# Bismarrck/tensoralloy

Measured on AMD Instinct MI355X. Metric: atom-steps/sec (energy+forces), 4000-atom Ni rcut=6.5 A, higher is better.
Workload: dtype f64

## Files before the change

### tensoralloy_amd/csrc/ta_api.hip

```cpp
#include <hip/hip_runtime.h>

#include <algorithm>
#include <chrono>
#include <climits>
#include <cmath>
#include <cstdio>
#include <cstdlib>
#include <cstring>
#include <stdexcept>
#include <string>
#include <vector>

#include "ta_device.h"
#include "ta_internal.h"
#include "ta_md.h"

namespace ta {
size_t mlp_scratch_doubles(const MlpDev &mlp);
void launch_mlp_impl(const MlpDev &mlp, int activation, int ndim, const int32_t *atoms, int n_atoms,
                     const DeviceBatch &b, double *scratch, hipStream_t s);
size_t mlp_all_scratch_doubles(const MlpDev *mlps_host, int nel, const int32_t *elem_start);
size_t td_scratch_doubles(const MlpDev *nets, int nel, int K, const int32_t *elem_start);
void launch_td_all(const MlpDev *nets_dev, const MlpDev *nets_host, int nel, int K, int act_h, int act,
                   int sommerfeld, int ndim, const DeviceBatch &b, const double *T, double *u_atom,
// ... 172 lines not shown
    if (n <= cap) return;
    if (ptr) HIP_CHECK(hipHostFree(ptr));
    ptr = nullptr;
    cap = 0;
    size_t want = n + n / 8 + 256;
    HIP_CHECK(hipHostMalloc((void **)&ptr, want, hipHostMallocDefault));
    cap = want;
  }
  void release() {
    if (ptr) (void)hipHostFree(ptr);
    ptr = nullptr;
    cap = 0;
  }
};

struct ChunkPlan {
  ta::AngChunk ch;
  int nb, ng, nz;
};

}

struct ta_context {
  int device = 0;
  hipStream_t stream = nullptr;
  hipStream_t own_stream = nullptr;
  int kind = 0;
  int n_elements = 0;
  int activation = 0;
  double rmax = 0.0;
  ta::SFParams sf;
  std::vector<ChunkPlan> chunks;
  std::vector<ChunkPlan> chunks_v2;
  bool use_v2 = false;
  ta::MlpDev *mlp_dev = nullptr;
  ta::MlpDev mlp[ta::kMaxElements];
  bool td = false, td_sommerfeld = false;
  int td_act = 0, td_K = 0;
  ta::MlpDev td_nets[3 * ta::kMaxElements];
  ta::MlpDev *td_dev = nullptr;
  std::vector<void *> model_allocs;
  ta::EamModel *eam = nullptr;
  ta::GrapModel *grap = nullptr;

  ta::HostPairs hp;
  ta::DeviceBatch db;
  bool have_batch = false;
  uint32_t last_want = 0;

  PinnedBuf stage_in, stage_out;
  DevBuf<char> inbuf;
  DevBuf<double> results;
  size_t o_blk = 0;
  DevBuf<double> rec, part4, G, dEdG, g, wat, bpart, fown, benergy, mlp_scratch;
  DevBuf<double> td_T, td_u, td_s;
  DevBuf<unsigned long long> masks;
  DevBuf<uint32_t> job_word;
  DevBuf<int32_t> job_count;
  DevBuf<uint32_t> job_word_own;
  DevBuf<int32_t> job_count_own;
  bool triangles = true;
  bool tri_cells_ok = false;
  int last_bwd_variant = 0;
  DevBuf<int32_t> pair_start, seg_start, pair_i, pair_j, pair_shift, pair_rev;
  ta::NlGrid *d_grids = nullptr;
  DevBuf<int32_t> nl_wrap, nl_binid, nl_bin_count, nl_bin_start, nl_bin_cursor, nl_bin_atoms, nl_counts;
  DevBuf<unsigned long long> nl_stats, nl_zero;
  unsigned long long *nl_stats_ptr = nullptr;
  bool nl_sorted = false;
  bool nl_rev_done = false;
  bool nl_zero_clean = false;
  int64_t nl_zero_atoms = -1;
  int nl_zero_bins = -1;
  DevBuf<double> hvp_buf;
#ifdef TA_PHASE_STAMPS
  DevBuf<unsigned long long> stamp_buf;
#endif
  DevBuf<ta::NlRec> nl_recs;
  bool pairs_on_device = false;
  bool descriptors_valid = false;
  DevBuf<double> train_scratch, train_partial, train_grad, train_coeff;
  DevBuf<double> jvp_J, tan_dD, tan_dG, tan_dir;
  DevBuf<double> filt_scratch;
  bool jvp_valid = false;

  double skin = 0.0;
  double r_list = 0.0;
  std::vector<int32_t> keep_species;
  std::vector<int32_t> keep_natoms, keep_pbc;
  std::vector<double> ref_pos, ref_cells;
  size_t o_pos = 0, o_cells = 0, o_species = 0;
  DevBuf<int32_t> ex_pair_i, ex_pair_j, ex_pair_shift, ex_pair_rev, ex_pair_start, ex_pair_stop, ex_seg_start, ex_counts,
      ex_map, ex_blk, ex_slot_q;
  bool filtered = false;
  bool upload_pending = false;
  bool mirror_next = false;
  uint32_t mirror_want = 0;
  int64_t n_list_builds = 0, n_list_reuses = 0;

  bool md_valid = false;
  DevBuf<double> md_mass, md_vel, md_ref, md_epot, md_ke;
  DevBuf<int32_t> md_blk_start;
  DevBuf<unsigned> md_status;
  PinnedBuf md_status_host;
  std::vector<int32_t> md_blk_start_host;
  int md_chunk = 0, md_n_blk = 0;
  int64_t md_ref_builds = -1;
// ... 456 lines not shown
  using namespace ta;
  if (h->nl_sorted) {
    nl_reverse_sorted(h->hp.n_pairs, h->n_elements, h->db.species, h->seg_start.ptr, h->pair_i.ptr,
                      h->pair_j.ptr, h->pair_shift.ptr, h->pair_rev.ptr, h->nl_stats_ptr, h->stream);
  } else {
    NlWork w = nl_work(h);
    nl_fill((int)h->hp.n_atoms, h->hp.n_pairs, h->n_elements, h->r_list, h->db.pos, h->db.species,
            h->db.frame_of_atom, h->d_grids, w, h->pair_i.ptr, h->pair_j.ptr, h->pair_shift.ptr,
            h->pair_rev.ptr, h->stream);
  }
  HIP_CHECK(hipGetLastError());
}

#ifdef TA_PHASE_STAMPS
static void dump_stamps(ta_context *h) {
  const char *path = std::getenv("TA_PHASE_STAMPS_OUT");
  if (!path || !h->db.stamps || h->db.n_blk <= 0) return;
  const size_t n = (size_t)2 * h->db.n_blk * 8;
  std::vector<unsigned long long> v(n);
  (void)hipStreamSynchronize(h->stream);
  (void)hipMemcpy(v.data(), h->db.stamps, n * sizeof(unsigned long long), hipMemcpyDeviceToHost);
  FILE *fp = std::fopen(path, "w");
  if (!fp) return;
  for (int k = 0; k < 2; ++k)
    for (int b = 0; b < h->db.n_blk; ++b) {
      std::fprintf(fp, "%d %d", k, b);
      for (int q = 0; q < 8; ++q) std::fprintf(fp, " %llu", v[((size_t)k * h->db.n_blk + b) * 8 + q]);
      std::fprintf(fp, "\n");
    }
  std::fclose(fp);
}
#endif

void launch_head(ta_context *h, const ta::DeviceBatch &db, hipStream_t s) {
  if (h->td)
    ta::launch_td_all(h->td_dev, h->td_nets, h->n_elements, h->td_K, h->td_act, h->activation,
                      h->td_sommerfeld ? 1 : 0, h->sf.ndim, db, h->td_T.ptr, h->td_u.ptr, h->td_s.ptr,
                      h->mlp_scratch.ptr, s);
  else
    ta::launch_mlp_all(h->mlp_dev, h->mlp, h->n_elements, h->activation, h->sf.ndim, db, h->mlp_scratch.ptr, s);
}

void compute_impl(ta_context *h, uint32_t want, bool timed, double *slot_ms) {
  using namespace ta;
#ifdef TA_PHASE_STAMPS
  if (h->db.n_blk > 0) {
    h->stamp_buf.ensure((size_t)2 * h->db.n_blk * 8 + 8);
    h->db.stamps = h->stamp_buf.ptr;
    (void)hipMemsetAsync(h->db.stamps, 0, (size_t)2 * h->db.n_blk * 8 * sizeof(unsigned long long), h->stream);
  }
#endif
  h->db.rec4 = nullptr;
  h->db.own_sums = 0;
  const DeviceBatch &db = h->db;
  hipStream_t s = h->stream;
  const bool need_forces = (want & (TA_WANT_FORCES | TA_WANT_VIRIAL)) != 0;
  auto begin = [&](int slot) {
    if (timed) HIP_CHECK(hipEventRecord(h->ev[2 * slot], s));
  };
  auto end = [&](int slot) {
    if (timed) HIP_CHECK(hipEventRecord(h->ev[2 * slot + 1], s));
  };
  bool used[TA_N_KERNEL_SLOTS] = {false};

  const bool has_mlp = h->kind == TA_MODEL_SF_MLP || h->kind == TA_MODEL_GRAP_MLP;
  if ((want & TA_WANT_REUSE_DESCRIPTORS) && has_mlp && h->descriptors_valid && !need_forces) {
    begin(TA_K_MLP);
    launch_head(h, db, s);
    end(TA_K_MLP);
    used[TA_K_MLP] = true;
  } else if (h->kind == TA_MODEL_SF_MLP) {
    static const bool full_records = getenv("TA_FULL_RECORDS") != nullptr;
    h->db.rec4 = (h->sf.angular && h->use_v2 && !full_records) ? h->db.rec : nullptr;
    if (!h->use_v2) {
      begin(TA_K_PAIR_GEOMETRY);
      launch_pair_geometry(h->sf, db, s);
      end(TA_K_PAIR_GEOMETRY);
      used[TA_K_PAIR_GEOMETRY] = true;
    }
    h->sf.ang_scale = h->use_v2 ? 1.0 : 0.5;
    const bool tri = h->use_v2 && h->triangles && h->tri_cells_ok && h->n_elements == 1 && need_forces;
    h->db.job_word_own = (tri && h->db.job_count) ? h->job_word_own.ptr : nullptr;
    h->db.job_count_own = (tri && h->db.job_count) ? h->job_count_own.ptr : nullptr;
    h->last_bwd_variant = 0;
    const bool reduce_in_forward = h->sf.angular && h->use_v2;
    if (h->sf.angular) {
      begin(TA_K_G4_FORWARD);
      if (h->use_v2) {
        bool geometry = true;
        size_t left = h->chunks_v2.size();
        for (const ChunkPlan &cp : h->chunks_v2) {
          --left;
          launch_g4_forward_v2(h->sf, cp.ch, cp.ng, cp.nz, geometry, left == 0, db, s);
          geometry = false;
        }
      } else
        for (const ChunkPlan &cp : h->chunks) launch_g4_forward(h->sf, cp.ch, cp.nb, cp.ng, cp.nz, db, s);
      end(TA_K_G4_FORWARD);
      used[TA_K_G4_FORWARD] = true;
    }
    if (!reduce_in_forward) {
      begin(TA_K_DESCRIPTOR_REDUCE);
      launch_descriptor_reduce(h->sf, db, s);
      end(TA_K_DESCRIPTOR_REDUCE);
      used[TA_K_DESCRIPTOR_REDUCE] = true;
    }
    begin(TA_K_MLP);
    launch_head(h, db, s);
    end(TA_K_MLP);
    used[TA_K_MLP] = true;
    if (need_forces) {
      begin(TA_K_BACKWARD);
      if (h->sf.angular) {
        bool first = true;
        if (h->use_v2)
          for (const ChunkPlan &cp : h->chunks_v2) {
            h->last_bwd_variant |= launch_backward_v2(h->sf, cp.ch, cp.ng, cp.nz, first, tri, db, s);
            first = false;
          }
        else
          for (const ChunkPlan &cp : h->chunks) {
            launch_backward(h->sf, cp.ch, cp.nb, cp.ng, cp.nz, first, false, db, s);
            first = false;
          }
      } else {
        AngChunk dummy;
        std::memset(&dummy, 0, sizeof(dummy));
        launch_backward(h->sf, dummy, 1, 1, 1, true, true, db, s);
      }
      end(TA_K_BACKWARD);
      used[TA_K_BACKWARD] = true;
      begin(TA_K_FORCE_GATHER);
      launch_force_gather(h->sf, db, s);
      end(TA_K_FORCE_GATHER);
      used[TA_K_FORCE_GATHER] = true;
    }
  } else if (h->kind == TA_MODEL_GRAP_MLP) {
    const bool net_exact = ta::grap_uses_filter_net(h->grap) && !ta::grap_filter_table_knots(h->grap);
    h->db.rec4 = (!net_exact && !getenv("TA_FULL_RECORDS")) ? h->db.rec : nullptr;
    begin(TA_K_GRAP);
    launch_grap_forward(h->grap, db, h->sf.eps, s);
    end(TA_K_GRAP);
    used[TA_K_GRAP] = true;
    begin(TA_K_MLP);
    launch_head(h, db, s);
    end(TA_K_MLP);
    used[TA_K_MLP] = true;
    if (need_forces) {
      begin(TA_K_BACKWARD);
      h->db.own_sums = getenv("TA_NO_OWN_SUMS") ? 0 : 1;
      launch_grap_backward(h->grap, db, s);
      end(TA_K_BACKWARD);
      used[TA_K_BACKWARD] = true;
      begin(TA_K_FORCE_GATHER);
      launch_force_gather(h->sf, db, s);
      end(TA_K_FORCE_GATHER);
      used[TA_K_FORCE_GATHER] = true;
    }
  } else {
    h->db.rec4 = getenv("TA_FULL_RECORDS") ? nullptr : h->db.rec;
    begin(TA_K_EAM);
    eam_compute(h->eam, db, want, s, nullptr);
    end(TA_K_EAM);
    used[TA_K_EAM] = true;
  }
  begin(TA_K_FRAME_REDUCE);
  {
    double *mirror = nullptr;
    int64_t n_tail = 0;
    h->mirror_want = 0;
    if (h->mirror_next && !timed) {
      const size_t N = (size_t)db.n_atoms, F = (size_t)db.n_frames;
      h->stage_out.ensure((10 * F + 4 * N + 2) * sizeof(double));
      mirror = reinterpret_cast<double *>(h->stage_out.ptr);
      n_tail = (int64_t)(need_forces ? 4 * N : N);
      h->mirror_want = want | TA_WANT_ENERGY | TA_WANT_ATOMIC;
    }
    launch_frame_reduce(db, need_forces, mirror, n_tail, s);
  }
  end(TA_K_FRAME_REDUCE);
  used[TA_K_FRAME_REDUCE] = true;
  HIP_CHECK(hipGetLastError());
  h->last_want = want;
  h->descriptors_valid = true;

  if (timed) {
    HIP_CHECK(hipStreamSynchronize(s));
    for (int k = 0; k < TA_N_KERNEL_SLOTS; ++k) {
      if (!used[k]) continue;
      float ms = 0.f;
      HIP_CHECK(hipEventElapsedTime(&ms, h->ev[2 * k], h->ev[2 * k + 1]));
      slot_ms[k] += ms;
    }
  }
}

template <typename F>
int guarded(ta_context *h, F &&fn) {
  try {
    if (h) HIP_CHECK(hipSetDevice(h->device));
    fn();
    return TA_OK;
  } catch (const HipError &e) {
    return fail(h, TA_ERR_HIP, e.what());
  } catch (const std::domain_error &e) {
    return fail(h, TA_ERR_UNSUPPORTED, e.what());
  } catch (const std::invalid_argument &e) {
    return fail(h, TA_ERR_INVALID, e.what());
  } catch (const std::bad_alloc &) {
    return fail(h, TA_ERR_NOMEM, "host allocation failed");
  } catch (const std::exception &e) {
    return fail(h, TA_ERR_INVALID, e.what());
  }
}

}

extern "C" {

int ta_abi_version(void) { return TA_ABI_VERSION; }
int ta_model_desc_size(void) { return (int)sizeof(ta_model_desc); }

int ta_device_count(void) {
  int n = 0;
  if (hipGetDeviceCount(&n) != hipSuccess) return 0;
  return n;
}

const char *ta_last_error(ta_handle h) { return h ? h->err.c_str() : g_create_error.c_str(); }

int ta_create(const ta_model_desc *model, int device, ta_handle *out) {
  if (!model || !out) return fail(nullptr, TA_ERR_INVALID, "null argument");
  *out = nullptr;
  int ndev = 0;
// ... 12 lines not shown
    if (std::strncmp(prop.gcnArchName, "gfx950", 6) != 0)
      throw HipError(std::string("device is ") + prop.gcnArchName +
                     ", this library is built for gfx950 only");
    HIP_CHECK(hipStreamCreateWithFlags(&h->own_stream, hipStreamNonBlocking));
    h->stream = h->own_stream;
    for (auto &e : h->ev) HIP_CHECK(hipEventCreate(&e));
    if (model->kind == TA_MODEL_SF_MLP) {
      build_sf_model(h, model);
    } else if (model->kind == TA_MODEL_GRAP_MLP) {
      if (model->cutoff_function != TA_CUTOFF_COSINE && model->cutoff_function != TA_CUTOFF_POLYNOMIAL)
        throw std::invalid_argument("unknown cutoff function");
      std::string err;
      h->grap = ta::grap_create(model, err);
      if (!h->grap) throw std::invalid_argument(err);
      h->rmax = model->rcut;
      std::memset(&h->sf, 0, sizeof(h->sf));
      h->sf.n_elements = model->n_elements;
      h->sf.eps = model->eps > 0.0 ? model->eps : 1e-14;
      h->sf.ndim = ta::grap_ndim(h->grap);
      build_mlp(h, model, h->sf.ndim);
    } else if (model->kind == TA_MODEL_EAM_ALLOY || model->kind == TA_MODEL_EAM_ADP || model->kind == TA_MODEL_EAM_FS) {
      std::string err;
      h->eam = ta::eam_create(model, err);
      if (!h->eam) throw std::invalid_argument(err);
      h->rmax = model->rcut;
      std::memset(&h->sf, 0, sizeof(h->sf));
      h->sf.n_elements = model->n_elements;
      h->sf.eps = model->eps > 0.0 ? model->eps : 1e-14;
    } else {
      throw std::invalid_argument("unknown model kind");
    }
  });
  if (rc != TA_OK) {
    g_create_error = h->err;
    ta_destroy(h);
    return rc;
  }
  *out = h;
  return TA_OK;
}

int ta_destroy(ta_handle h) {
  if (!h) return TA_OK;
  (void)hipSetDevice(h->device);
#ifdef TA_PHASE_STAMPS
  dump_stamps(h);
#endif
  if (h->stream) (void)hipStreamSynchronize(h->stream);
  for (void *p : h->model_allocs) (void)hipFree(p);
  if (h->eam) ta::eam_destroy(h->eam);
  if (h->grap) ta::grap_destroy(h->grap);
  h->stage_in.release(); h->stage_out.release(); h->inbuf.release(); h->results.release();
  h->rec.release(); h->part4.release(); h->G.release();
  h->dEdG.release(); h->g.release(); h->wat.release(); h->bpart.release(); h->fown.release();
  h->benergy.release(); h->mlp_scratch.release();
  h->train_scratch.release(); h->train_partial.release(); h->train_grad.release(); h->train_coeff.release();
  h->jvp_J.release(); h->tan_dD.release(); h->tan_dG.release(); h->tan_dir.release();
  h->pair_start.release(); h->seg_start.release(); h->pair_i.release(); h->pair_j.release();
  h->pair_shift.release(); h->pair_rev.release();
  for (auto *b : {&h->ex_pair_i, &h->ex_pair_j, &h->ex_pair_shift, &h->ex_pair_rev, &h->ex_pair_start, &h->ex_pair_stop,
                  &h->ex_seg_start, &h->ex_counts, &h->ex_map, &h->ex_blk, &h->ex_slot_q})
    b->release();
  h->masks.release(); h->job_word.release(); h->job_count.release();
  h->job_word_own.release(); h->job_count_own.release();
  for (auto *b : {&h->nl_wrap, &h->nl_binid, &h->nl_bin_count, &h->nl_bin_start, &h->nl_bin_cursor,
                  &h->nl_bin_atoms, &h->nl_counts})
    b->release();
  h->nl_stats.release();
  h->nl_zero.release();
  h->hvp_buf.release();
  h->filt_scratch.release();
  h->nl_recs.release();
  for (auto *b : {&h->md_mass, &h->md_vel, &h->md_ref, &h->md_epot, &h->md_ke, &h->md_noise}) b->release();
  h->md_blk_start.release();
  h->md_status.release();
  h->md_status_host.release();
  for (auto &e : h->ev)
    if (e) (void)hipEventDestroy(e);
  if (h->own_stream) (void)hipStreamDestroy(h->own_stream);
  delete h;
  return TA_OK;
}

}

namespace {
void ensure_job_lists(ta_context *h, size_t n_blk) {
  static const bool off = std::getenv("TA_NO_JOBS") != nullptr;
  if (off || !h->use_v2 || n_blk == 0) {
    h->db.job_count = nullptr;
    return;
  }
  const int stride = ta::v2_job_stride(h->db.cap);
  h->job_word.ensure(n_blk * (size_t)stride + 8);
  h->job_count.ensure(n_blk + 8);
  if (h->n_elements == 1) {
    h->job_word_own.ensure(n_blk * (size_t)stride + 8);
    h->job_count_own.ensure(n_blk + 8);
  }
  h->db.job_word = h->job_word.ptr;
  h->db.job_count = h->job_count.ptr;
  h->db.job_stride = stride;
}

bool filter_applies(const ta_context *h) {
  if (!(h->skin > 0.0) || h->hp.n_atoms == 0 || std::getenv("TA_NO_LIST_FILTER")) return false;
  if (h->kind == TA_MODEL_SF_MLP) return h->use_v2;
  if (h->kind == TA_MODEL_EAM_ALLOY || h->kind == TA_MODEL_EAM_FS) return ta::eam_is_plain(h->eam);
  return false;
}

void apply_filter(ta_context *h) {
  using namespace ta;
  const size_t N = (size_t)h->hp.n_atoms, P = (size_t)h->hp.n_pairs;
  const int nel = h->n_elements;
  h->ex_pair_i.ensure(P + 1);
  h->ex_pair_j.ensure(P + 1);
  h->ex_pair_shift.ensure(3 * P + 3);
  h->ex_pair_rev.ensure(P + 1);
  h->ex_pair_start.ensure(N + 1);
  h->ex_pair_stop.ensure(N + 1);
  h->ex_seg_start.ensure(N * (nel + 1) + 1);
  h->ex_map.ensure(P + 1);
  const int n_run_slots = nl_filter_blocks((int)N);
  h->ex_blk.ensure((size_t)n_run_slots + 4);
  const bool blocks = h->kind == TA_MODEL_SF_MLP;
  const bool indirect = blocks && !std::getenv("TA_FILTER_REV_KERNEL");
  if (indirect) h->ex_slot_q.ensure(P + 1);
  nl_filter((int)N, (int64_t)P, nel, h->rmax, h->db.pos, h->db.cells, h->db.frame_of_atom,
            h->pair_start.ptr, h->seg_start.ptr, h->pair_j.ptr, h->pair_shift.ptr, h->pair_rev.ptr, h->ex_map.ptr,
            h->ex_seg_start.ptr, h->ex_pair_start.ptr, h->ex_pair_stop.ptr, h->ex_pair_i.ptr, h->ex_pair_j.ptr,
            h->ex_pair_shift.ptr, h->ex_pair_rev.ptr, indirect ? h->ex_slot_q.ptr : nullptr, h->db.cap,
            blocks ? h->ex_blk.ptr : nullptr, h->stream);
  h->db.slot_q = indirect ? h->ex_slot_q.ptr : nullptr;
  h->db.rev_super = indirect ? h->pair_rev.ptr : nullptr;
  h->db.rev_map = indirect ? h->ex_map.ptr : nullptr;
  HIP_CHECK(hipGetLastError());
  h->db.pair_start = h->ex_pair_start.ptr;
  h->db.pair_stop = h->ex_pair_stop.ptr;
  h->db.seg_start = h->ex_seg_start.ptr;
// ... 1779 lines not shown
```

### tensoralloy_amd/csrc/ta_device.h

```cpp
#pragma once
#include <hip/hip_runtime.h>

#include <cstdint>

#include "tensoralloy_amd.h"

namespace ta {

constexpr int kMaxRadial = 64;
constexpr int kMaxElements = 8;
constexpr int kMaxBetaSlots = 3;
constexpr int kRecDoubles = 8;
constexpr int kMaxLayers = 8;
constexpr int kCapMin = 192;
constexpr int kCapMax = 1024;
constexpr int kMaxCentersPerBlock = 16;
constexpr int kMaxHd = 24;

struct SFParams {
  double rcut, acut;
  double inv_rc2, inv_ac2;
  double two_inv_ac2;
  double eps;
  double ang_scale;
// ... 15 lines not shown
  int hslot[2];
  double gamma[2];
  double zeta[2];
  double kz[2];
  int zeta_int[2];
  int chan[8];
  int safe_pow;
  int n_hd;
  double hd[kMaxHd];
};

struct DeviceBatch {
  int64_t n_atoms = 0, n_pairs = 0;
  int n_frames = 0, nnl_max = 0;
  double *pos = nullptr;
  double *cells = nullptr;
  int32_t *species = nullptr;
  int32_t *frame_of_atom = nullptr;
  int32_t *atom_start = nullptr;
  int32_t *pair_start = nullptr;
  int32_t *pair_stop = nullptr;
  int32_t *seg_start = nullptr;
  int32_t *pair_i = nullptr, *pair_j = nullptr, *pair_shift = nullptr, *pair_rev = nullptr;
  const int32_t *slot_q = nullptr, *rev_super = nullptr, *rev_map = nullptr;
  int32_t *blk_center = nullptr;
  int n_blk = 0;
  int blk_groups = 0;
  const int32_t *n_blk_dev = nullptr;
  int cap = kCapMin;
  int32_t *elem_atoms = nullptr;
  int32_t elem_start[kMaxElements + 1] = {0};

  double *rec = nullptr;
  double *rec4 = nullptr;
  double *part4 = nullptr;
  unsigned long long *masks = nullptr;
  uint32_t *job_word = nullptr;
  int32_t *job_count = nullptr;
  int job_stride = 0;
  uint32_t *job_word_own = nullptr;
  int32_t *job_count_own = nullptr;
  double *G = nullptr;
  double *dEdG = nullptr;
  double *eatom = nullptr;
  double *g = nullptr;
  double *forces = nullptr;
  double *wat = nullptr;
  double *fown = nullptr;
  int own_sums = 0;
#ifdef TA_PHASE_STAMPS
  unsigned long long *stamps = nullptr;
#endif
  double *bpart = nullptr;
  double *energy = nullptr;
  double *virial = nullptr;
  double *batch_energy = nullptr;
};

__host__ __device__ inline int triangle_owner_rank(uint32_t index_sum) {
#ifdef __HIP_DEVICE_COMPILE__
  const uint32_t h = __umul24(index_sum, 0x9E3779u);
#else
  const uint32_t h = index_sum * 0x9E3779u;
#endif
  return (int)(((h & 0xFFFFFFu) * 3u) >> 24);
}
__host__ __device__ inline bool owns_triangle(int32_t i, int32_t j, int32_t k) {
  return triangle_owner_rank((uint32_t)i + (uint32_t)j + (uint32_t)k) == (j < i ? 1 : 0) + (k < i ? 1 : 0);
}

#ifdef __HIPCC__
__device__ __forceinline__ int pair_stop_of(const DeviceBatch &b, int64_t i) {
  return b.pair_stop ? b.pair_stop[i] : b.pair_start[i + 1];
}
#endif

#ifdef __HIPCC__
__device__ __forceinline__ int pair_rev_of(const DeviceBatch &b, int q) {
  return b.slot_q ? b.rev_map[b.rev_super[b.slot_q[q]]] : b.pair_rev[q];
}
__device__ __forceinline__ const double2 *pair_geom(const DeviceBatch &b, size_t q) {
  return reinterpret_cast<const double2 *>(b.rec4 ? b.rec4 + 4 * q : b.rec + kRecDoubles * q);
}
#endif

struct MlpLayerDev {
  int k, n;
  int kp, np;
  double *w;
  double *wt;
  double *b;
  int act;
  int res;
};
struct MlpDev {
  int n_layers = 0;
  MlpLayerDev layer[kMaxLayers];
  double *xlo = nullptr, *xhi = nullptr;
  int max_np = 0, max_kp = 0;
};

void launch_pair_geometry(const SFParams &sf, const DeviceBatch &b, hipStream_t s);
void launch_g4_forward(const SFParams &sf, const AngChunk &ch, int nb, int ng, int nz,
                       const DeviceBatch &b, hipStream_t s);
void launch_descriptor_reduce(const SFParams &sf, const DeviceBatch &b, hipStream_t s);
void launch_mlp(const SFParams &sf, const MlpDev &mlp, int activation, int element,
                const DeviceBatch &b, hipStream_t s);
void launch_backward(const SFParams &sf, const AngChunk &ch, int nb, int ng, int nz,
                     bool first, bool radial_only, const DeviceBatch &b, hipStream_t s);
void launch_force_gather(const SFParams &sf, const DeviceBatch &b, hipStream_t s);
void launch_frame_reduce(const DeviceBatch &b, bool want_virial, double *mirror, int64_t n_tail, hipStream_t s);

size_t g4_lds_bytes(int nnl_max);

size_t v2_lds_bytes(bool backward, int cap, int n_local = 0, int nspec = 0, bool triangles = false);
int v2_job_stride(int cap);
void launch_g4_forward_v2(const SFParams &sf, const AngChunk &ch, int ng, int nz, bool geometry,
                          bool reduce, const DeviceBatch &b, hipStream_t s);
int launch_backward_v2(const SFParams &sf, const AngChunk &ch, int ng, int nz, bool first, bool triangles,
                       const DeviceBatch &b, hipStream_t s);

struct NlGrid {
  double h[9];
  double hinv[9];
  double lo[3];
  double inv_w[3];
  int32_t nb[3];
  int32_t pbc[3];
  int32_t bin_offset;
  int32_t pad_;
  int32_t m[3];
  int32_t ortho;
  double bw[3];
};
struct NlRec {
  double x, y, z;
  int32_t wx, wy, wz;
  int32_t j;
  int32_t sp;
  int32_t pad_;
};
struct NlWork {
  int32_t *wrap;
  int32_t *binid;
  int32_t *bin_count;
  int32_t *bin_start;
  int32_t *bin_cursor;
  int32_t *bin_atoms;
  NlRec *recs;
  int32_t *counts;
  int32_t *seg_start;
  unsigned long long *stats;
};
bool nl_make_grid(const ta_frame &fr, double rmax, int bin_offset, NlGrid &g);
int nl_bins(const NlGrid &g);
void nl_count(int n_atoms, int n_bins, int nel, double rmax, const double *pos, const int32_t *species,
              const int32_t *frame_of_atom, const NlGrid *grids, NlWork &w, int32_t *pair_start,
              hipStream_t s);
size_t nl_build_zero_words(int n_atoms, int n_bins);
void nl_build(int n_atoms, int n_bins, int nel, double rmax, const double *pos, const int32_t *species,
              const int32_t *frame_of_atom, const NlGrid *grids, NlWork &w, unsigned long long *zero,
              bool zero_is_clean, long long capacity, int32_t *pair_start, int32_t *host_pair_start,
              int32_t *pair_i, int32_t *pair_j, int32_t *pair_shift, int32_t *pair_rev, long long rev_cover,
              hipStream_t s);
void nl_reverse_sorted(int64_t n_pairs, int nel, const int32_t *species, const int32_t *seg_start,
                       const int32_t *pair_i, const int32_t *pair_j, const int32_t *pair_shift,
                       int32_t *pair_rev, unsigned long long *stats, hipStream_t s);
int nl_filter_blocks(int n_atoms);
void nl_filter(int n_atoms, int64_t n_super, int nel, double rmax, const double *pos, const double *cells,
               const int32_t *frame_of_atom, const int32_t *start_super, const int32_t *seg_super,
               const int32_t *pj_super, const int32_t *ps_super, const int32_t *rev_super, int32_t *map,
               int32_t *seg_exact, int32_t *pair_start, int32_t *pair_stop, int32_t *pi_out, int32_t *pj_out,
               int32_t *ps_out, int32_t *rev_out, int32_t *slot_q, int cap, int32_t *blk_center, hipStream_t s);
// ... 6 lines not shown
```

### tensoralloy_amd/csrc/ta_kernels.hip

```cpp
#include <hip/hip_runtime.h>

#include <algorithm>

#include <cstdlib>
#include <stdexcept>

#include "ta_device.h"
#include "ta_math.h"
#include "ta_reduce.h"

namespace ta {

namespace {

constexpr int kBlock = 256;

__device__ __forceinline__ int radial_term(int center, int other) {
  return other == center ? 0 : (other < center ? other + 1 : other);
}
__device__ __forceinline__ int angular_term(int s1, int s2, int nel) {
  int a = s1 < s2 ? s1 : s2, b = s1 < s2 ? s2 : s1;
  return a * nel - (a * (a - 1)) / 2 + (b - a);
}

// ... 213 lines not shown
      double fd, dfd;
      cutoff_u(sf.cutoff, u, fd, dfd);
      double A = 0.0, Q = 0.0;
#pragma unroll
      for (int ib = 0; ib < NB; ++ib) {
        const double ed = ta_exp(-ch.beta[ib] * u);
        const double Hb = rb[5 + ch.hslot[ib]];
        const double Hd = ed * fd;
        const double Hd2 = 2.0 * sf.inv_ac2 * ed * (dfd - ch.beta[ib] * fd);
        double S0 = 0.0, S1 = 0.0;
#pragma unroll
        for (int ig = 0; ig < NG; ++ig) {
          const double base = fma(ch.gamma[ig], cth, 1.0);
#pragma unroll
          for (int iz = 0; iz < NZ; ++iz) {
            double pm1;
            if (ch.zeta_int[iz] > 0)
              pm1 = pow_int_m1(base, ch.zeta_int[iz]);
            else
              pm1 = safe_pow_grad(ch.safe_pow, base, ch.zeta[iz] - 1.0);
            S0 = fma(w[ib][ig][iz], pm1 * base, S0);
            S1 = fma(w[ib][ig][iz] * ch.zeta[iz] * ch.gamma[ig], pm1, S1);
          }
        }
        A = fma(Hb * Hd, fma(S1 * Ha[ib], inv_ab - cth * inv_ra2, S0 * Ga[ib]), A);
        Q = fma(Ha[ib] * Hb, fma(-S1 * inv_ab, Hd, S0 * Hd2), Q);
      }
      A = ok ? A : 0.0;
      Q = ok ? Q : 0.0;
      sumAQ += A + Q;
      vx = fma(Q, bx, vx);
      vy = fma(Q, by, vy);
      vz = fma(Q, bz, vz);
    }
  }
  double gx = fma(ax, sumAQ, -vx), gy = fma(ay, sumAQ, -vy), gz = fma(az, sumAQ, -vz);
  if (first) {
    double s;
    radial_backward(sf, b, i, sa, ra2, inv_ra, s);
    s *= inv_ra;
    gx = fma(s, ax, gx);
    gy = fma(s, ay, gy);
    gz = fma(s, az, gz);
  } else {
    gx += b.g[4 * (size_t)p];
    gy += b.g[4 * (size_t)p + 1];
    gz += b.g[4 * (size_t)p + 2];
  }
  b.g[4 * (size_t)p] = gx;
  b.g[4 * (size_t)p + 1] = gy;
  b.g[4 * (size_t)p + 2] = gz;
}

template <int W>
__global__ __launch_bounds__(16 * W) void force_gather_kernel(DeviceBatch b) {
  const int64_t i = ((int64_t)blockIdx.x * (16 * W) + threadIdx.x) / W;
  const int lane = threadIdx.x & (W - 1);
  const bool active = i < b.n_atoms;
  double f[3] = {0, 0, 0}, w[9] = {0, 0, 0, 0, 0, 0, 0, 0, 0};
  const int q0 = active ? b.pair_start[i] : 0, q1 = active ? pair_stop_of(b, i) : 0;
  if (b.own_sums) {
    for (int qb = q0 + lane; qb < q1; qb += 4 * W) {
      int r[4];
      bool ok[4];
#pragma unroll
      for (int k = 0; k < 4; ++k) {
        const int q = qb + W * k;
        ok[k] = q < q1;
        r[k] = ok[k] ? pair_rev_of(b, q) : 0;
      }
      double gr[4][3];
#pragma unroll
      for (int k = 0; k < 4; ++k) {
        const double2 *grp = reinterpret_cast<const double2 *>(b.g + 4 * (size_t)r[k]);
        const double2 c0 = grp[0], c1 = grp[1];
        gr[k][0] = c0.x;
        gr[k][1] = c0.y;
        gr[k][2] = c1.x;
      }
#pragma unroll
      for (int k = 0; k < 4; ++k)
        if (ok[k]) {
          f[0] -= gr[k][0];
          f[1] -= gr[k][1];
          f[2] -= gr[k][2];
        }
    }
#pragma unroll
    for (int k = 0; k < 3; ++k) f[k] = group_sum<W>(f[k]);
    if (lane == 0 && active) {
      const double *own = b.fown + 12 * (size_t)i;
      for (int k = 0; k < 3; ++k) b.forces[3 * (size_t)i + k] = f[k] + own[k];
      for (int k = 0; k < 9; ++k) w[k] = own[3 + k];
    }
    block_partials(b, blockIdx.x, i, active, lane == 0, w);
    return;
  }
  for (int qb = q0 + lane; qb < q1; qb += 4 * W) {
    int r[4];
    bool ok[4];
#pragma unroll
    for (int k = 0; k < 4; ++k) {
      const int q = qb + W * k;
      ok[k] = q < q1;
      r[k] = ok[k] ? pair_rev_of(b, q) : 0;
    }
    double gq[4][3], gr[4][3], d[4][3];
#pragma unroll
// ... 132 lines not shown
  return (size_t)(kBlock + 2 * (size_t)nnl_max) * kRecDoubles * sizeof(double);
}

void launch_pair_geometry(const SFParams &sf, const DeviceBatch &b, hipStream_t s) {
  if (b.n_pairs == 0) return;
  hipLaunchKernelGGL(pair_geometry_kernel, dim3(blocks_for(b.n_pairs, kBlock)), dim3(kBlock), 0, s,
                     sf, b);
}

#define TA_DISPATCH(FN, ...)                                             \
  do {                                                                   \
    const int key = nb * 100 + ng * 10 + nz;                             \
    switch (key) {                                                       \
      case 111: FN<1, 1, 1>(__VA_ARGS__); break;                         \
      case 112: FN<1, 1, 2>(__VA_ARGS__); break;                         \
      case 121: FN<1, 2, 1>(__VA_ARGS__); break;                         \
      case 122: FN<1, 2, 2>(__VA_ARGS__); break;                         \
      case 211: FN<2, 1, 1>(__VA_ARGS__); break;                         \
      case 212: FN<2, 1, 2>(__VA_ARGS__); break;                         \
      case 221: FN<2, 2, 1>(__VA_ARGS__); break;                         \
      case 222: FN<2, 2, 2>(__VA_ARGS__); break;                         \
      default: throw std::domain_error("no angular kernel for this (beta, gamma, zeta) chunk shape"); \
    }                                                                    \
  } while (0)

void launch_g4_forward(const SFParams &sf, const AngChunk &ch, int nb, int ng, int nz,
                       const DeviceBatch &b, hipStream_t s) {
  if (b.n_pairs == 0) return;
  TA_DISPATCH(launch_fwd_t, sf, ch, b, s);
}

void launch_descriptor_reduce(const SFParams &sf, const DeviceBatch &b, hipStream_t s) {
  if (b.n_atoms == 0) return;
  hipLaunchKernelGGL(descriptor_reduce_kernel, dim3(blocks_for(b.n_atoms * 64, kBlock)),
                     dim3(kBlock), 0, s, sf, b);
}

void launch_backward(const SFParams &sf, const AngChunk &ch, int nb, int ng, int nz, bool first,
                     bool radial_only, const DeviceBatch &b, hipStream_t s) {
  if (b.n_pairs == 0) return;
  if (radial_only) {
    hipLaunchKernelGGL(g2_backward_kernel, dim3(blocks_for(b.n_pairs, kBlock)), dim3(kBlock), 0, s,
                       sf, b);
    return;
  }
  const int f = first ? 1 : 0;
  TA_DISPATCH(launch_bwd_t, sf, ch, b, f, s);
}

void launch_force_gather(const SFParams &, const DeviceBatch &b, hipStream_t s) {
  if (b.n_atoms == 0) return;
  static const int w_env = getenv("TA_GATHER_W") ? atoi(getenv("TA_GATHER_W")) : 0;
  const int W = (w_env == 16 || w_env == 32) ? w_env : (b.n_atoms < 16384 ? 32 : 16);
  const dim3 grid((unsigned)((b.n_atoms + 15) / 16));
  if (W == 32) hipLaunchKernelGGL(force_gather_kernel<32>, grid, dim3(512), 0, s, b);
  else hipLaunchKernelGGL(force_gather_kernel<16>, grid, dim3(256), 0, s, b);
}

void launch_frame_reduce(const DeviceBatch &b, bool want_virial, double *mirror, int64_t n_tail, hipStream_t s) {
  if (b.n_frames == 0) return;
  const unsigned extra = (mirror && n_tail > 0) ? (unsigned)std::min<int64_t>((n_tail + kRedBlock - 1) / kRedBlock, 32) : 0u;
  hipLaunchKernelGGL(frame_reduce_kernel, dim3((unsigned)b.n_frames + extra), dim3(kRedBlock), 0, s, b,
                     want_virial ? 1 : 0, want_virial ? 1 : 0, mirror, (long long)(mirror ? n_tail : 0));
  if (b.n_frames > 1) hipLaunchKernelGGL(batch_energy_kernel, dim3(1), dim3(kBlock), 0, s, b);
}

}
```

### tensoralloy_amd/csrc/ta_kernels_v2.hip

```cpp
#include <hip/hip_runtime.h>

#include <cstdio>
#include <cstdlib>
#include <stdexcept>
#include <type_traits>

#include "ta_device.h"
#include "ta_math.h"
#include "ta_reduce.h"

namespace ta {
namespace {

constexpr int kBlock = 256;
constexpr int kNF = 8;
constexpr int kNFf = 7;
constexpr int kSegW = 6;
constexpr int kOwnCtl = 60 + 2 * kMaxCentersPerBlock * kSegW;
constexpr int kJobCtlBytes = (kOwnCtl + 40) * 4;
__host__ __device__ inline int v2_pcols(int cap, int nspec) {
  return nspec >= 1 ? cap / 4 + kMaxCentersPerBlock * nspec : cap;
}
constexpr int kRingPad = 64;
constexpr int kRTab = 8;
// ... 772 lines not shown
        __syncthreads();
      }
      return;
    }
    if (active) run_item(item, true, mask, nullptr, nullptr, std::false_type{});
    }
  } else {
    if (b.job_count && threadIdx.x == 0) b.job_count[blockIdx.x] = -1;
    if (jidx && threadIdx.x == 0) b.job_count_own[blockIdx.x] = -1;
    for (int it = threadIdx.x; it < M; it += blockDim.x) run_item(it, false, 0ull, nullptr, nullptr, std::false_type{});
  }

  if (flags & 2) {
    __syncthreads();
    const int ncent = c1 - c0;
    const int nwaves = blockDim.x >> 6;
    if (ncent <= nwaves) {
      const int w = threadIdx.x >> 6, l = threadIdx.x & 63;
      const bool act = w < ncent;
      const int64_t i = c0 + (act ? w : 0);
      atom_descriptors<64>(sf, b, i, l, act, [&](int c, double v) { b.G[(size_t)i * sf.ndim + c] = v; });
    } else {
      const int row = threadIdx.x >> 4, l = threadIdx.x & 15, nrows = blockDim.x >> 4;
      for (int k0 = 0; k0 < ncent; k0 += nrows) {
        const bool act = k0 + row < ncent;
        const int64_t i = c0 + (act ? k0 + row : 0);
        atom_descriptors<16>(sf, b, i, l, act, [&](int c, double v) { b.G[(size_t)i * sf.ndim + c] = v; });
      }
    }
  }
}

template <int NSPEC, int NG, int NZ, int HD, bool DEFZ, int CAP, int WPE = (DEFZ ? (NSPEC <= 2 ? 5 : 4) : 0),
          bool TRI = false>
__global__ __launch_bounds__(kBlock)
    __attribute__((amdgpu_waves_per_eu(WPE > 0 ? WPE : 1, 8))) void backward_v2_kernel(SFParams sf, AngChunk ch,
                                                             DeviceBatch b, int flags) {
  static_assert(!DEFZ || NZ == 2, "DEFZ needs the two-zeta grid");
  static_assert(!TRI || (NSPEC == 1 && DEFZ && HD > 0), "the triangle build is one-element, default grid, Hd series");
  const int first = flags & 1;
  if (b.n_blk_dev && (int)blockIdx.x >= *b.n_blk_dev) return;
  stagger(flags);
  extern __shared__ double lds[];
  const int kCap = CAP > 0 ? CAP : b.cap;
  const Fields f = carve(lds, kCap);
  double *gacc = lds + kNF * kCap + kCap / 8;
  const int slot = b.blk_groups > 0 ? 16 * ((int)blockIdx.x % b.blk_groups) + (int)blockIdx.x / b.blk_groups
                                    : (int)blockIdx.x;
  const int c0 = b.blk_center[slot], c1 = b.blk_center[slot + 1];
  if (c0 >= c1) return;
  const int s0 = b.pair_start[c0];
  const int M = pair_stop_of(b, c1 - 1) - s0;
  const double beta = ch.beta[0];
  for (int k = threadIdx.x; k < 3 * kCap; k += blockDim.x) gacc[k] = 0.0;
  int *cstart = reinterpret_cast<int *>(gacc) - 20;
  if ((int)threadIdx.x <= c1 - c0 && threadIdx.x < 17)
    cstart[threadIdx.x] = ((int)threadIdx.x < c1 - c0 ? b.pair_start[c0 + threadIdx.x] : s0 + M) - s0;
  double *pctab = gacc + 3 * kCap;
  if constexpr (DEFZ && NSPEC == 1) {
    const int k = (int)blockDim.x - 1 - (int)threadIdx.x;
    if (k < c1 - c0) {
      const double *wsrc = b.dEdG + (size_t)(c0 + k) * sf.ndim + sf.n_radial_dim;
      double p0 = 0.0, p1 = 0.0, p2 = 0.0, p3 = 0.0, p4 = 0.0;
#pragma unroll
      for (int ig = 0; ig < NG; ++ig) {
        const double g1 = ch.gamma[ig], g2 = g1 * g1;
        const double w1 = wsrc[ch.chan[ig * NZ]] * ch.kz[0], w4 = wsrc[ch.chan[ig * NZ + 1]] * ch.kz[1];
        p0 += w1 + w4;
        p1 += g1 * (w1 + 4.0 * w4);
        p2 += 6.0 * g2 * w4;
        p3 += 4.0 * g2 * g1 * w4;
        p4 += g2 * g2 * w4;
      }
      pctab[5 * k] = p0;
      pctab[5 * k + 1] = 0.5 * p1;
      pctab[5 * k + 2] = 0.25 * p2;
      pctab[5 * k + 3] = 0.125 * p3;
      pctab[5 * k + 4] = 0.0625 * p4;
    }
  }
  double *rtab = pctab + 5 * kMaxCentersPerBlock;
  const bool use_rtab = first && NSPEC * sf.n_rad <= kRTab;
  if (use_rtab) {
    const int per = NSPEC * sf.n_rad;
    const int t = (int)blockDim.x - 1 - (int)threadIdx.x - kMaxCentersPerBlock;
    if (t >= 0 && t < (c1 - c0) * per) {
      const int ci = t / per, rem = t - ci * per;
      const int sb = rem / sf.n_rad, c = rem - sb * sf.n_rad;
      const int64_t i = c0 + ci;
      rtab[ci * kRTab + rem] = b.dEdG[(size_t)i * sf.ndim + radial_term2(b.species[i], sb) * sf.n_rad + c];
    }
  }
  double2 *pn01 = reinterpret_cast<double2 *>(rtab + kMaxCentersPerBlock * kRTab), *pn23 = pn01 + kCap;
  double *pn4 = reinterpret_cast<double *>(pn23 + kCap);
  if constexpr (TRI) {
    for (int item = threadIdx.x; item < M; item += blockDim.x) {
      double pc[5];
      defz_coeffs<NG, NZ>(ch, b.dEdG + (size_t)b.pair_j[s0 + item] * sf.ndim + sf.n_radial_dim, pc);
      pn01[item] = make_double2(pc[0], pc[1]);
      pn23[item] = make_double2(pc[2], pc[3]);
      pn4[item] = pc[4];
    }
  }
  TA_STAMP(b, 1, 0);
  stage<HD>(sf, ch, beta, b, f, s0, M);
  TA_STAMP(b, 1, 1);
// ... 305 lines not shown
        if constexpr (TRI) run_tri(item, true, mask, std::false_type{});
        else run_item(item, true, mask, std::false_type{});
      }
    } else {
      for (int it = threadIdx.x; it < M; it += blockDim.x) {
        if constexpr (TRI) run_tri(it, false, 0ull, std::false_type{});
        else run_item(it, false, 0ull, std::false_type{});
      }
    }
  }
  __syncthreads();
  TA_STAMP(b, 1, 4);
  for (int item = threadIdx.x; item < M; item += blockDim.x) {
    const int64_t p = (int64_t)s0 + item;
    double gx = gacc[item], gy = gacc[kCap + item], gz = gacc[2 * kCap + item];
    if (first) {
      const double *wr;
      if (use_rtab) {
        int ci = 0;
        for (int k = 1; k < c1 - c0; ++k) ci += (item >= cstart[k]) ? 1 : 0;
        wr = rtab + ci * kRTab + (NSPEC == 1 ? 0 : (int)f.gs[item].y * sf.n_rad);
      } else {
        const int i = b.pair_i[p];
        wr = b.dEdG + (size_t)i * sf.ndim + radial_term2(b.species[i], (int)f.gs[item].y) * sf.n_rad;
      }
      const double r2 = f.zr[item].y, inv_r = f.ih[item].x;
      const double ur = r2 * sf.inv_rc2;
      double s = 0.0;
      if (ur < 1.0) {
        double fc, dfdu;
        cutoff_u(sf.cutoff, ur, fc, dfdu);
        const double r = r2 * inv_r;
        const double dfdr = dfdu * 2.0 * r * sf.inv_rc2;
        double e = 0.0;
        for (int c = 0; c < sf.n_rad; ++c) {
          const double dr = r - sf.omega[c];
          const int pw = sf.eta_pow[c];
          e = pw > 0 ? pow_int_m1(e, pw) * e : ta_exp(-sf.eta[c] * dr * dr * sf.inv_rc2);
          s = fma(wr[c], e * (dfdr - 2.0 * sf.eta[c] * dr * fc * sf.inv_rc2), s);
        }
      }
      s *= inv_r;
      gx = fma(s, f.xy[item].x, gx);
      gy = fma(s, f.xy[item].y, gy);
      gz = fma(s, f.zr[item].x, gz);
    } else {
      gx += b.g[4 * (size_t)p];
      gy += b.g[4 * (size_t)p + 1];
      gz += b.g[4 * (size_t)p + 2];
    }
    b.g[4 * (size_t)p] = gx;
    b.g[4 * (size_t)p + 1] = gy;
    b.g[4 * (size_t)p + 2] = gz;
  }
  TA_STAMP(b, 1, 5);
}

template <int NSPEC, int NG, int NZ>
void fwd_t(const SFParams &sf, const AngChunk &ch, const DeviceBatch &b, int geom, hipStream_t s) {
  const dim3 grid((unsigned)b.n_blk), block((unsigned)(b.cap < kBlock ? b.cap : kBlock));
  const size_t lds = v2_lds_bytes(false, b.cap, b.job_count ? NSPEC * NG * NZ : 0, NSPEC);
  if constexpr (NZ == 2) {
    if (ch.n_hd == 12 && ch.zeta_int[0] == 1 && ch.zeta_int[1] == 4) {
      if (b.cap == kCapMin) {
        static const int force = getenv("TA_FWD_WPE") ? atoi(getenv("TA_FWD_WPE")) : 0;
        if constexpr (NSPEC <= 2) {
          if (force != 5) {
            hipLaunchKernelGGL((g4_forward_v2_kernel<NSPEC, NG, NZ, 12, true, kCapMin, 6>), grid, block, lds, s, sf, ch,
                               b, geom);
            return;
          }
        }
        hipLaunchKernelGGL((g4_forward_v2_kernel<NSPEC, NG, NZ, 12, true, kCapMin>), grid, block, lds, s, sf, ch, b, geom);
      } else
        hipLaunchKernelGGL((g4_forward_v2_kernel<NSPEC, NG, NZ, 12, true, 0>), grid, block, lds, s, sf, ch, b, geom);
      return;
    }
    if (ch.n_hd == 16 && ch.zeta_int[0] == 1 && ch.zeta_int[1] == 4) {
      hipLaunchKernelGGL((g4_forward_v2_kernel<NSPEC, NG, NZ, 16, true, 0>), grid, block, lds, s, sf, ch, b, geom);
      return;
    }
  }
  if (ch.n_hd > 0 && ch.n_hd <= 16)
    hipLaunchKernelGGL((g4_forward_v2_kernel<NSPEC, NG, NZ, 16, false, 0>), grid, block, lds, s, sf, ch, b, geom);
  else if (ch.n_hd == 24)
    hipLaunchKernelGGL((g4_forward_v2_kernel<NSPEC, NG, NZ, 24, false, 0>), grid, block, lds, s, sf, ch, b, geom);
  else
    hipLaunchKernelGGL((g4_forward_v2_kernel<NSPEC, NG, NZ, 0, false, 0>), grid, block, lds, s, sf, ch, b, geom);
}
template <int NSPEC, int NG, int NZ>
void bwd_t(const SFParams &sf, const AngChunk &ch, const DeviceBatch &b, int first, bool tri, int &variant,
           hipStream_t s) {
  const dim3 grid((unsigned)b.n_blk), block((unsigned)(b.cap < kBlock ? b.cap : kBlock));
  const size_t lds = v2_lds_bytes(true, b.cap);
  variant = 1;
  if constexpr (NZ == 2 && NSPEC == 1) {
    if (tri && (ch.n_hd == 12 || ch.n_hd == 16) && ch.zeta_int[0] == 1 && ch.zeta_int[1] == 4) {
      const size_t lds_t = v2_lds_bytes(true, b.cap, 0, 0, true);
      variant = 2;
      static const int force = getenv("TA_BWD_WPE") ? atoi(getenv("TA_BWD_WPE")) : 0;
      if (ch.n_hd == 12 && b.cap == kCapMin && force == 4)
        hipLaunchKernelGGL((backward_v2_kernel<1, NG, NZ, 12, true, kCapMin, 4, true>), grid, block, lds_t, s, sf, ch,
                           b, first);
      else if (ch.n_hd == 12 && b.cap == kCapMin)
        hipLaunchKernelGGL((backward_v2_kernel<1, NG, NZ, 12, true, kCapMin, 5, true>), grid, block, lds_t, s, sf, ch,
                           b, first);
// ... 51 lines not shown
#define TA_DISPATCH_V2(FN, ...)                                   \
  do {                                                            \
    const int key = nspec * 100 + ng * 10 + nz;                   \
    if (key == 122) FN<1, 2, 2>(__VA_ARGS__);                     \
    else if (key == 222) FN<2, 2, 2>(__VA_ARGS__);                \
    else throw std::domain_error("TA_V2_FEW build");              \
  } while (0)
#else
#define TA_DISPATCH_V2(FN, ...)                                   \
  do {                                                            \
    const int key = nspec * 100 + ng * 10 + nz;                   \
    switch (key) {                                                \
      case 111: FN<1, 1, 1>(__VA_ARGS__); break;                  \
      case 112: FN<1, 1, 2>(__VA_ARGS__); break;                  \
      case 121: FN<1, 2, 1>(__VA_ARGS__); break;                  \
      case 122: FN<1, 2, 2>(__VA_ARGS__); break;                  \
      case 211: FN<2, 1, 1>(__VA_ARGS__); break;                  \
      case 212: FN<2, 1, 2>(__VA_ARGS__); break;                  \
      case 221: FN<2, 2, 1>(__VA_ARGS__); break;                  \
      case 222: FN<2, 2, 2>(__VA_ARGS__); break;                  \
      case 311: FN<3, 1, 1>(__VA_ARGS__); break;                  \
      case 312: FN<3, 1, 2>(__VA_ARGS__); break;                  \
      case 321: FN<3, 2, 1>(__VA_ARGS__); break;                  \
      case 322: FN<3, 2, 2>(__VA_ARGS__); break;                  \
      case 422: FN<4, 2, 2>(__VA_ARGS__); break;                  \
      case 522: FN<5, 2, 2>(__VA_ARGS__); break;                  \
      default:                                                    \
        throw std::domain_error("no second-generation angular kernel for this (species, gamma, zeta) shape"); \
    }                                                             \
  } while (0)
#endif

static int stagger_bits(const DeviceBatch &b, const char *var) {
  const char *e = getenv(var);
  if (getenv("TA_DEBUG_NO_TRIPLES")) return 1 << 24;
  if (const char *d = getenv("TA_DEBUG_SKIP")) return (atoi(d) & 127) << 24;
  if (!e) return 0;
  int n = 0, shift = 3;
  if (sscanf(e, "%d,%d", &n, &shift) < 1) return 0;
  (void)b;
  return ((n & 0xff) << 8) | ((shift & 31) << 16);
}

void launch_g4_forward_v2(const SFParams &sf, const AngChunk &ch, int ng, int nz, bool geometry,
                          bool reduce, const DeviceBatch &b, hipStream_t s) {
  if (b.n_blk == 0) return;
  const int nspec = sf.n_elements;
  const int geom = (geometry ? 1 : 0) | (reduce ? 2 : 0) | ((geometry && reduce) ? 4 : 0) |
                   stagger_bits(b, "TA_STAGGER_FWD");
  TA_DISPATCH_V2(fwd_t, sf, ch, b, geom, s);
}

int launch_backward_v2(const SFParams &sf, const AngChunk &ch, int ng, int nz, bool first, bool triangles,
                       const DeviceBatch &b, hipStream_t s) {
  if (b.n_blk == 0) return 0;
  const int nspec = sf.n_elements;
  const int f = (first ? 1 : 0) | stagger_bits(b, "TA_STAGGER_BWD");
  int variant = 0;
  TA_DISPATCH_V2(bwd_t, sf, ch, b, f, triangles, variant, s);
  return variant;
}

}
```

Before: 36.94 million.

## Compute per-block virial records in backward and fold frame sums into force gather

```diff
diff --git a/tensoralloy_amd/csrc/ta_api.hip b/tensoralloy_amd/csrc/ta_api.hip
--- a/tensoralloy_amd/csrc/ta_api.hip
+++ b/tensoralloy_amd/csrc/ta_api.hip
@@ -248,7 +248,7 @@
   DevBuf<char> inbuf;
   DevBuf<double> results;
   size_t o_blk = 0;
-  DevBuf<double> rec, part4, G, dEdG, g, wat, bpart, fown, benergy, mlp_scratch;
+  DevBuf<double> rec, part4, G, dEdG, g, wat, bpart, brec, fown, benergy, mlp_scratch;
   DevBuf<double> td_T, td_u, td_s;
   DevBuf<unsigned long long> masks;
   DevBuf<uint32_t> job_word;
@@ -811,6 +811,7 @@
 #endif
   h->db.rec4 = nullptr;
   h->db.own_sums = 0;
+  h->db.frame_recs = 0;
   const DeviceBatch &db = h->db;
   hipStream_t s = h->stream;
   const bool need_forces = (want & (TA_WANT_FORCES | TA_WANT_VIRIAL)) != 0;
@@ -869,15 +870,23 @@
     end(TA_K_MLP);
     used[TA_K_MLP] = true;
     if (need_forces) {
+      if (h->sf.angular && h->use_v2 && !h->chunks_v2.empty() && db.n_blk > 0 && db.n_atoms > 0 &&
+          db.n_atoms < 16384 && !(h->mirror_next && !timed)) {
+        h->db.brec = h->brec.ptr;
+        h->db.frame_recs = 1;
+      }
       begin(TA_K_BACKWARD);
       if (h->sf.angular) {
         bool first = true;
-        if (h->use_v2)
+        if (h->use_v2) {
+          size_t left = h->chunks_v2.size();
           for (const ChunkPlan &cp : h->chunks_v2) {
-            h->last_bwd_variant |= launch_backward_v2(h->sf, cp.ch, cp.ng, cp.nz, first, tri, db, s);
+            --left;
+            h->last_bwd_variant |= launch_backward_v2(h->sf, cp.ch, cp.ng, cp.nz, first, tri, db, s,
+                                                      left == 0 && db.frame_recs != 0);
             first = false;
           }
-        else
+        } else
           for (const ChunkPlan &cp : h->chunks) {
             launch_backward(h->sf, cp.ch, cp.nb, cp.ng, cp.nz, first, false, db, s);
             first = false;
@@ -923,7 +932,8 @@
     end(TA_K_EAM);
     used[TA_K_EAM] = true;
   }
-  begin(TA_K_FRAME_REDUCE);
+  const bool sums_in_gather = db.frame_recs != 0 && db.n_frames == 1;
+  if (!sums_in_gather) begin(TA_K_FRAME_REDUCE);
   {
     double *mirror = nullptr;
     int64_t n_tail = 0;
@@ -937,8 +947,8 @@
     }
     launch_frame_reduce(db, need_forces, mirror, n_tail, s);
   }
-  end(TA_K_FRAME_REDUCE);
-  used[TA_K_FRAME_REDUCE] = true;
+  if (!sums_in_gather) end(TA_K_FRAME_REDUCE);
+  used[TA_K_FRAME_REDUCE] = !sums_in_gather;
   HIP_CHECK(hipGetLastError());
   h->last_want = want;
   h->descriptors_valid = true;
@@ -1057,7 +1067,7 @@
   if (h->grap) ta::grap_destroy(h->grap);
   h->stage_in.release(); h->stage_out.release(); h->inbuf.release(); h->results.release();
   h->rec.release(); h->part4.release(); h->G.release();
-  h->dEdG.release(); h->g.release(); h->wat.release(); h->bpart.release(); h->fown.release();
+  h->dEdG.release(); h->g.release(); h->wat.release(); h->bpart.release(); h->brec.release(); h->fown.release();
   h->benergy.release(); h->mlp_scratch.release();
   h->train_scratch.release(); h->train_partial.release(); h->train_grad.release(); h->train_coeff.release();
   h->jvp_J.release(); h->tan_dD.release(); h->tan_dG.release(); h->tan_dir.release();
@@ -1091,6 +1101,7 @@
 
 namespace {
 void ensure_job_lists(ta_context *h, size_t n_blk) {
+  if (h->use_v2) h->brec.ensure(9 * n_blk + 9);
   static const bool off = std::getenv("TA_NO_JOBS") != nullptr;
   if (off || !h->use_v2 || n_blk == 0) {
     h->db.job_count = nullptr;
diff --git a/tensoralloy_amd/csrc/ta_device.h b/tensoralloy_amd/csrc/ta_device.h
--- a/tensoralloy_amd/csrc/ta_device.h
+++ b/tensoralloy_amd/csrc/ta_device.h
@@ -91,6 +91,8 @@
   unsigned long long *stamps = nullptr;
 #endif
   double *bpart = nullptr;
+  double *brec = nullptr;
+  int frame_recs = 0;
   double *energy = nullptr;
   double *virial = nullptr;
   double *batch_energy = nullptr;
@@ -157,7 +159,7 @@
 void launch_g4_forward_v2(const SFParams &sf, const AngChunk &ch, int ng, int nz, bool geometry,
                           bool reduce, const DeviceBatch &b, hipStream_t s);
 int launch_backward_v2(const SFParams &sf, const AngChunk &ch, int ng, int nz, bool first, bool triangles,
-                       const DeviceBatch &b, hipStream_t s);
+                       const DeviceBatch &b, hipStream_t s, bool records = false);
 
 struct NlGrid {
   double h[9];
diff --git a/tensoralloy_amd/csrc/ta_kernels.hip b/tensoralloy_amd/csrc/ta_kernels.hip
--- a/tensoralloy_amd/csrc/ta_kernels.hip
+++ b/tensoralloy_amd/csrc/ta_kernels.hip
@@ -289,8 +289,117 @@
   b.g[4 * (size_t)p + 2] = gz;
 }
 
+template <int T>
+__device__ __forceinline__ void frame_sums_from_records(const DeviceBatch &b, int f) {
+  __shared__ double red[10][T / 64];
+  const int tid = threadIdx.x;
+  const int a0 = b.atom_start[f], a1 = b.atom_start[f + 1];
+  double acc[10];
+#pragma unroll
+  for (int k = 0; k < 10; ++k) acc[k] = 0.0;
+  for (int a = a0 + tid; a < a1; a += T) acc[0] += b.eatom[a];
+  const int n_live = b.n_blk_dev ? *b.n_blk_dev : b.n_blk;
+  int lo = 0, hi = b.n_blk;
+  if (b.n_frames > 1 && !b.n_blk_dev) {
+    int l = 0, r = b.n_blk;
+    while (l < r) {
+      const int m = (l + r) >> 1;
+      if (b.blk_center[m + 1] > a0) r = m;
+      else l = m + 1;
+    }
+    lo = l;
+    r = b.n_blk;
+    while (l < r) {
+      const int m = (l + r) >> 1;
+      if (b.blk_center[m] >= a1) r = m;
+      else l = m + 1;
+    }
+    hi = l;
+  }
+  for (int sl = lo + tid; sl < hi; sl += T) {
+    if (b.n_blk_dev) {
+      const int wg = b.blk_groups > 0 ? (sl & 15) * b.blk_groups + (sl >> 4) : sl;
+      if (wg >= n_live) continue;
+    }
+    const int c0 = b.blk_center[sl], c1 = b.blk_center[sl + 1];
+    if (c0 >= c1) continue;
+    if (c0 >= a0 && c1 <= a1) {
+      const double *p = b.brec + 9 * (size_t)sl;
+#pragma unroll
+      for (int k = 0; k < 9; ++k) acc[1 + k] += p[k];
+    } else {
+      for (int a = max(c0, a0); a < min(c1, a1); ++a)
+        for (int k = 0; k < 9; ++k) acc[1 + k] += b.wat[9 * (size_t)a + k];
+    }
+  }
+  const int lane = tid & 63, wave = tid >> 6;
+#pragma unroll
+  for (int k = 0; k < 10; ++k) {
+    const double v = wave_sum(acc[k]);
+    if (lane == 0) red[k][wave] = v;
+  }
+  __syncthreads();
+  if (tid < 10) {
+    double v = 0.0;
+    for (int w = 0; w < T / 64; ++w) v += red[tid][w];
+    if (tid == 0) {
+      b.energy[f] = v;
+      if (b.n_frames == 1) b.batch_energy[0] = v;
+    } else {
+      b.virial[9 * (size_t)f + (tid - 1)] = v;
+    }
+  }
+}
+
 template <int W>
 __global__ __launch_bounds__(16 * W) void force_gather_kernel(DeviceBatch b) {
+  if (b.frame_recs) {
+    if ((int)blockIdx.x < b.n_frames) {
+      frame_sums_from_records<16 * W>(b, (int)blockIdx.x);
+      return;
+    }
+    const int64_t i = ((int64_t)((int)blockIdx.x - b.n_frames) * (16 * W) + threadIdx.x) / W;
+    const int lane = threadIdx.x & (W - 1);
+    const bool active = i < b.n_atoms;
+    double f[3] = {0, 0, 0};
+    const int q0 = active ? b.pair_start[i] : 0, q1 = active ? pair_stop_of(b, i) : 0;
+    for (int qb = q0 + lane; qb < q1; qb += 4 * W) {
+      int r[4];
+      bool ok[4];
+#pragma unroll
+      for (int k = 0; k < 4; ++k) {
+        const int q = qb + W * k;
+        ok[k] = q < q1;
+        r[k] = ok[k] ? pair_rev_of(b, q) : 0;
+      }
+      double gq[4][3], gr[4][3];
+#pragma unroll
+      for (int k = 0; k < 4; ++k) {
+        const int q = ok[k] ? qb + W * k : q0;
+        const double2 *gqp = reinterpret_cast<const double2 *>(b.g + 4 * (size_t)q);
+        const double2 *grp = reinterpret_cast<const double2 *>(b.g + 4 * (size_t)r[k]);
+        const double2 a0 = gqp[0], a1 = gqp[1], c0 = grp[0], c1 = grp[1];
+        gq[k][0] = a0.x;
+        gq[k][1] = a0.y;
+        gq[k][2] = a1.x;
+        gr[k][0] = c0.x;
+        gr[k][1] = c0.y;
+        gr[k][2] = c1.x;
+      }
+#pragma unroll
+      for (int k = 0; k < 4; ++k) {
+        if (!ok[k]) continue;
+#pragma unroll
+        for (int c = 0; c < 3; ++c) f[c] += gq[k][c] - gr[k][c];
+      }
+    }
+#pragma unroll
+    for (int k = 0; k < 3; ++k) f[k] = group_sum<W>(f[k]);
+    if (lane == 0 && active) {
+      for (int k = 0; k < 3; ++k) b.forces[3 * (size_t)i + k] = f[k];
+    }
+    return;
+  }
   const int64_t i = ((int64_t)blockIdx.x * (16 * W) + threadIdx.x) / W;
   const int lane = threadIdx.x & (W - 1);
   const bool active = i < b.n_atoms;
@@ -529,13 +638,17 @@
   if (b.n_atoms == 0) return;
   static const int w_env = getenv("TA_GATHER_W") ? atoi(getenv("TA_GATHER_W")) : 0;
   const int W = (w_env == 16 || w_env == 32) ? w_env : (b.n_atoms < 16384 ? 32 : 16);
-  const dim3 grid((unsigned)((b.n_atoms + 15) / 16));
+  const dim3 grid((unsigned)((b.n_atoms + 15) / 16) + (b.frame_recs ? (unsigned)b.n_frames : 0u));
   if (W == 32) hipLaunchKernelGGL(force_gather_kernel<32>, grid, dim3(512), 0, s, b);
   else hipLaunchKernelGGL(force_gather_kernel<16>, grid, dim3(256), 0, s, b);
 }
 
 void launch_frame_reduce(const DeviceBatch &b, bool want_virial, double *mirror, int64_t n_tail, hipStream_t s) {
   if (b.n_frames == 0) return;
+  if (b.frame_recs) {
+    if (b.n_frames > 1) hipLaunchKernelGGL(batch_energy_kernel, dim3(1), dim3(kBlock), 0, s, b);
+    return;
+  }
   const unsigned extra = (mirror && n_tail > 0) ? (unsigned)std::min<int64_t>((n_tail + kRedBlock - 1) / kRedBlock, 32) : 0u;
   hipLaunchKernelGGL(frame_reduce_kernel, dim3((unsigned)b.n_frames + extra), dim3(kRedBlock), 0, s, b,
                      want_virial ? 1 : 0, want_virial ? 1 : 0, mirror, (long long)(mirror ? n_tail : 0));
diff --git a/tensoralloy_amd/csrc/ta_kernels_v2.hip b/tensoralloy_amd/csrc/ta_kernels_v2.hip
--- a/tensoralloy_amd/csrc/ta_kernels_v2.hip
+++ b/tensoralloy_amd/csrc/ta_kernels_v2.hip
@@ -848,6 +848,8 @@
   const int s0 = b.pair_start[c0];
   const int M = pair_stop_of(b, c1 - 1) - s0;
   const double beta = ch.beta[0];
+  const bool records = (flags & 2) != 0;
+  const bool straddles = records && b.frame_of_atom[c0] != b.frame_of_atom[c1 - 1];
   for (int k = threadIdx.x; k < 3 * kCap; k += blockDim.x) gacc[k] = 0.0;
   int *cstart = reinterpret_cast<int *>(gacc) - 20;
   if ((int)threadIdx.x <= c1 - c0 && threadIdx.x < 17)
@@ -1259,6 +1261,49 @@
     b.g[4 * (size_t)p] = gx;
     b.g[4 * (size_t)p + 1] = gy;
     b.g[4 * (size_t)p + 2] = gz;
+    if (records) {
+      gacc[item] = gx;
+      gacc[kCap + item] = gy;
+      gacc[2 * kCap + item] = gz;
+    }
+  }
+  if (records) {
+    double *red = pctab;
+    const int lane = threadIdx.x & 63, wave = threadIdx.x >> 6;
+#pragma unroll 1
+    for (int c = 0; c < 3; ++c) {
+      double wx = 0.0, wy = 0.0, wz = 0.0;
+      for (int item = threadIdx.x; item < M; item += blockDim.x) {
+        const double gc = gacc[c * kCap + item];
+        const double2 dxy = f.xy[item];
+        wx = fma(gc, dxy.x, wx);
+        wy = fma(gc, dxy.y, wy);
+        wz = fma(gc, f.zr[item].x, wz);
+      }
+      wx = wave_sum(wx);
+      wy = wave_sum(wy);
+      wz = wave_sum(wz);
+      if (lane == 0) {
+        red[4 * (3 * c) + wave] = wx;
+        red[4 * (3 * c + 1) + wave] = wy;
+        red[4 * (3 * c + 2) + wave] = wz;
+      }
+    }
+    __syncthreads();
+    if (threadIdx.x < 9) {
+      double v = 0.0;
+      for (int w = 0; w < (int)(blockDim.x >> 6); ++w) v += red[4 * threadIdx.x + w];
+      b.brec[9 * (size_t)slot + threadIdx.x] = v;
+    }
+    if (straddles && (int)threadIdx.x < 9 * (c1 - c0)) {
+      const int ci = (int)threadIdx.x / 9, k = (int)threadIdx.x - 9 * ci, c = k / 3, e = k - 3 * c;
+      double v = 0.0;
+      for (int q = cstart[ci]; q < cstart[ci + 1]; ++q) {
+        const double d = e == 0 ? f.xy[q].x : (e == 1 ? f.xy[q].y : f.zr[q].x);
+        v = fma(gacc[c * kCap + q], d, v);
+      }
+      b.wat[9 * (size_t)(c0 + ci) + k] = v;
+    }
   }
   TA_STAMP(b, 1, 5);
 }
@@ -1416,10 +1461,10 @@
 }
 
 int launch_backward_v2(const SFParams &sf, const AngChunk &ch, int ng, int nz, bool first, bool triangles,
-                       const DeviceBatch &b, hipStream_t s) {
+                       const DeviceBatch &b, hipStream_t s, bool records) {
   if (b.n_blk == 0) return 0;
   const int nspec = sf.n_elements;
-  const int f = (first ? 1 : 0) | stagger_bits(b, "TA_STAGGER_BWD");
+  const int f = (first ? 1 : 0) | (records ? 2 : 0) | stagger_bits(b, "TA_STAGGER_BWD");
   int variant = 0;
   TA_DISPATCH_V2(bwd_t, sf, ch, b, f, triangles, variant, s);
   return variant;
```

Result: no change. 37.11 million (median of 6 runs) (+0.5%).
